# gam0022/hanamaru-renderer

Hardware: AMD Instinct MI355X
Metric: Mpaths/sec at 1920x1080x1024spp (rtcamp6 scene); achieved GB/s in BVH traversal (higher is better)
Workload: dtype f32

## Files before the change

hanamaru-renderer_amd/csrc/device_scene.h:

```cpp
#pragma once
#include <math.h>
#include <stdint.h>

#if defined(__HIPCC__)
#define HD __host__ __device__ __forceinline__
#else
#define HD inline
#endif

namespace hr {

struct alignas(16) f4 { float x, y, z, w; };

struct alignas(16) Node {
    float nearx, neary, farx, fary;
    float nearz, farz;
    uint32_t a;
    uint32_t b;
};
HD void node_set_box(Node &n, const float *mn, const float *mx, int octant) {
    n.nearx = (octant & 1) ? mx[0] : mn[0]; n.farx = (octant & 1) ? mn[0] : mx[0];
    n.neary = (octant & 2) ? mx[1] : mn[1]; n.fary = (octant & 2) ? mn[1] : mx[1];
    n.nearz = (octant & 4) ? mx[2] : mn[2]; n.farz = (octant & 4) ? mn[2] : mx[2];
}
// ... 174 lines not shown
    uint32_t tail_div;
    uint32_t wg_budget;
    GovDev *gov;
    uint64_t rec_lo_off;
    uint32_t org_x, org_y, reg_w, reg_h;
    const uint32_t *tile_list;
    uint32_t tile_count;
};
HD uint32_t rp_reg_w(const RenderParams &rp) { return rp.reg_w ? rp.reg_w : rp.width; }
HD uint32_t rp_reg_h(const RenderParams &rp) { return rp.reg_h ? rp.reg_h : rp.height; }
HD bool rp_in_region(const RenderParams &rp, uint32_t px, uint32_t py) { return px < rp_reg_w(rp) && py < rp_reg_h(rp); }

HD void tile_lane_pixel(const RenderParams &rp, uint32_t tile, uint32_t j, uint32_t &px, uint32_t &py, uint32_t &sub) {
    uint32_t tx = tile % rp.tiles_x, ty = tile / rp.tiles_x;
    uint32_t pix = j >> 2;
    sub = j & 3u;
    px = tx * 4u + (pix & 3u);
    py = ty * 4u + (pix >> 2);
}
HD void tile_lane_frame_pixel(const RenderParams &rp, uint32_t tile, uint32_t j, uint32_t &px, uint32_t &py, uint32_t &sub) {
    tile_lane_pixel(rp, tile, j, px, py, sub);
    px += rp.org_x;
    py += rp.org_y;
}

static const int ISAAC_TAIL = 64;
static const int REC_FLOATS = 32;
static const int REC_DRAWS = 28;
static const int REC_HEAD = 28;
static const int LENS_FAST = 5;
static const int DRAWS_PER_PATH = 20;
static const uint32_t REC_ITEM_FLOATS = 64u * REC_FLOATS;
static const int SEG_B1 = 11, SEG_B2 = 21, SEG_NBLK = 11;
HD uint32_t rec_slot(uint32_t lane_base, uint32_t slot) { return lane_base + (slot >> 2) * 256u + (slot & 3u); }

struct Counters {
    unsigned long long paths, rays, node_tests, tri_tests, sphere_tests, cuboid_tests, rng_overflow, shadow_culled;
    unsigned long long shade_calls, shade_lanes, box_passes, box_lanes, leaf_calls, leaf_lanes, outer_iters, pad2;
    unsigned long long phase_cycles[4];
    unsigned long long seed_phase[8];
};

}
```

hanamaru-renderer_amd/csrc/hr_api.hip:

```cpp
#include <hip/hip_runtime.h>

#include <cmath>
#include <cstdarg>
#include <cstdio>
#include <cstring>
#include <map>
#include <mutex>
#include <string>
#include <vector>

#include "bvh_build.h"
#include "device_scene.h"
#include "flatten.h"
#include "gpu_bvh.h"
#include "hanamaru_hip.h"
#include "hanamaru_hip_debug.h"
#include "hr_comm.h"
#include "isaac_core.h"
#include "post_core.h"
#include "pt_core.h"

using namespace hr;


// ... 87 lines not shown
    uint32_t ovf_cap = 0;
    u64 *ovf_win = nullptr;
    size_t draws_cap = 0;
    uint64_t rec_lo_off = 0;
    int draw_residuals = 1;
    u64 *ring = nullptr;
    int seed_split = 16;
    uint32_t init_prio = 1;
    hipEvent_t seed_done[2] = {nullptr, nullptr}, trace_done[2] = {nullptr, nullptr};
    bool seed_pending[2] = {false, false}, trace_pending[2] = {false, false};
    uint64_t batch_counter = 0;
    Counters *d_counters = nullptr;
    uint32_t *d_tile_counter = nullptr;
    bool counters = false;
    uint32_t batch = 0;
    uint32_t adv_den = 2, leaf_den = 2;
    int min_waves = 5;
    uint32_t trace_wgs = 6;
    uint32_t tail_div = 16;
    uint32_t trace_grid = 0, trace_budget = 0;
    uint32_t node_unroll = 2;
    uint32_t kchunk = 0;
    int trace_boost = -1;
    GovDev *gov = nullptr;
    bool quant_nodes = true;
    int max_leaf = 4;
    double split_ratio = -1.0;
    int bvh_builder = -1;
    int builder_in_use = 0;
    double bvh_build_ms = 0;
    uint64_t max_tail_bytes = 20ull << 30;
    int seed_mode = 2;
    int seed_prof = 0;
    uint32_t seed_prio = 3;
    uint32_t nee_cull = 7;
    uint32_t rr_start = 0;
    uint32_t ploc_top = hr::lbvh::PLOC_TOP_CLUSTERS;
    int trace_mode = 0;
    int trace_mode_opt = -1;
    int precise_opt = -1;
    bool precise = false;
    bool wf_has_prec = false;
    WfQueues wf{};
    void *wf_block = nullptr;
    uint32_t wf_adv_den = 2, wf_trav_wgs = 8, wf_shade_wgs = 8;
    int debug_skip = 0;
    std::vector<EventPair> seed_events, trace_events, post_events, debug_events;
    double seed_ms = 0, trace_ms = 0, post_ms = 0, debug_ms = 0;
    uint64_t seed_launches = 0, trace_launches = 0, debug_launches = 0;
    uint64_t paths_rendered = 0;
    std::vector<std::pair<uint64_t, hipEvent_t>> markers;
    uint64_t next_ticket = 1;
};

static std::mutex g_bound_mu;
static std::map<const void *, std::pair<const hr_ctx *, size_t>> g_bound;
static void unbind_accumulator(hr_ctx *c) {
    std::lock_guard<std::mutex> lk(g_bound_mu);
    for (auto it = g_bound.begin(); it != g_bound.end();) it = it->second.first == c ? g_bound.erase(it) : std::next(it);
}
static void free_scene(hr_ctx *c) {
    for (void *p : c->scene_allocs) (void)hipFree(p);
    c->scene_allocs.clear();
    c->have_scene = false;
}
template <class T>
// ... 746 lines not shown
    return HR_OK;
}
static int launch_split(hr_ctx *c, const RenderParams &rp, int slot, std::vector<hipEvent_t> *marks = nullptr, uint32_t *plog = nullptr, const WfQueues *queues = nullptr) {
    const WfQueues wq = queues ? *queues : c->wf;
    hipStream_t st = c->stream;
    auto mark = [&]() -> hipError_t { if (!marks) return hipSuccess; hipEvent_t e; hipError_t r = hipEventCreate(&e); if (r != hipSuccess) return r; marks->push_back(e); return hipEventRecord(e, st); };
    const bool log = plog != nullptr;
    const WfStartFn start = select_wf_start_kernel(c->precise, rp.tile_list != nullptr);
    const WfTraverseFn traverse = select_wf_traverse_kernel(c->counters, c->dsc.qnodes != nullptr, log);
    const WfShadeFn shade = select_wf_shade_kernel(c->counters, c->precise, log);
    if (!start || !traverse || !shade) return fail(HR_ERR_UNSUPPORTED, "split pipeline: no kernel instantiation for these options (kernel_variants.h)");
    HIP_TRY(hipMemsetAsync(wq.counts, 0, (WF_STEPS + 2) * WF_SUBQ * sizeof(WfCounts), st));
    HIP_TRY(mark());
    auto grid_of = [&](uint32_t wgs_per_cu) { return dim3(std::max<uint32_t>(16u, (uint32_t)c->num_cus * wgs_per_cu / 16u * 16u)); };
    hipLaunchKernelGGL(start, grid_of(8u), dim3(256), 0, st, c->dsc, rp, c->recs[slot], wq);
    HIP_TRY(mark());
    RenderParams rt = rp;
    rt.adv_den = c->wf_adv_den;
    const dim3 gt = grid_of(c->wf_trav_wgs), gs = grid_of(c->wf_shade_wgs), b(256);
    for (uint32_t step = 1; step <= WF_STEPS; step++) {
        hipLaunchKernelGGL(traverse, gt, b, 0, st, c->dsc, rt, wq, step, c->d_counters);
        HIP_TRY(mark());
        hipLaunchKernelGGL(shade, gs, b, 0, st, c->dsc, rp, c->recs[slot], wq, step, c->d_counters, plog);
        HIP_TRY(mark());
    }
    HIP_TRY(hipGetLastError());
    return HR_OK;
}

static int launch_seed(hr_ctx *c, const RenderParams &rp, int slot, hipStream_t st) {
    const bool list = rp.tile_list != nullptr;
    uint64_t paths = (uint64_t)(list ? rp.tile_count : rp.tiles_x * rp.tiles_y) * rp.num_k * 64u;
    uint32_t grid = (uint32_t)std::min<uint64_t>((paths + SEED_COLS - 1) / SEED_COLS, (uint64_t)c->num_cus);
    const SeedVariant *v = select_seed_kernel(c->seed_mode, c->seed_split, c->seed_prof, rp.rec_lo_off != 0, list);
    if (!v) return fail(HR_ERR_UNSUPPORTED, "no seed kernel instantiation for seed_mode %d, seed_split %d, seed_prof %d%s (kernel_variants.h)", c->seed_mode, c->seed_split, c->seed_prof, list ? " under a tile mask" : "");
    const bool skip = (c->debug_skip & 2) != 0;
    if (!skip && v->ring && !c->ring) HIP_TRY(hipMalloc((void **)&c->ring, (size_t)c->num_cus * SEED_RING_WORDS_MAX * sizeof(u64)));
    EventPair ev;
    HIP_TRY(timed_begin(ev, st));
    hipError_t e = hipSuccess;
    if (!skip) {
        RenderParams krp = rp;
        int lens_shape = c->dsc.cam.lens_shape;
        void *args[7] = {&krp, &lens_shape, &c->ring, &c->recs[slot], &c->ovf, &c->ovf_win, &c->d_counters};
        if (!v->ring) std::copy(args + 3, args + 7, args + 2);
        e = hipLaunchKernel(v->fn, dim3(grid), dim3(v->threads), args, SEED_LDS_BYTES, st);
    }
    HIP_TRY(timed_end(e, ev, st, c->seed_events, &c->seed_launches));
    return HR_OK;
}

static void target_params(const hr_ctx *c, RenderParams &rp) {
    rp.width = c->W; rp.height = c->H;
    rp.org_x = c->RX; rp.org_y = c->RY; rp.reg_w = c->RW; rp.reg_h = c->RH;
    rp.tiles_x = (c->RW + 3) / 4; rp.tiles_y = (c->RH + 3) / 4;
}
static void knob_params(const hr_ctx *c, RenderParams &rp) {
    rp.adv_den = c->adv_den; rp.leaf_den = c->leaf_den;
    rp.node_unroll = c->node_unroll; rp.kchunk = c->kchunk;
    rp.nee_cull_off = ~c->nee_cull & 7u;
}
static uint32_t render_batch(const hr_ctx *c, uint32_t tiles, bool split) {
    uint64_t batch = c->batch;
    if (!batch) {
        const uint64_t per_sampling_paths = (uint64_t)tiles * 64u;
        batch = std::min<uint64_t>(64, std::max<uint64_t>(4, (33177600ull + per_sampling_paths - 1) / per_sampling_paths));
    }
// ... 746 lines not shown
    constexpr OptionField(int hr_ctx::*p) : i(p) {}
};
enum { OPT_SYNC = 1, OPT_GOVERN = 2 };
struct OptionRow {
    const char *key;
    OptionField field;
    double lo, hi, step;
    const char *error;
    int flags;
};
static const OptionRow PRODUCT_OPTIONS[] = {
    {"counters", &hr_ctx::counters, 1, 0, 0, "", 0},
    {"batch", &hr_ctx::batch, 0, 64, 0, "batch must be in [1,64], or 0 for automatic", OPT_SYNC},
    {"trace_boost", &hr_ctx::trace_boost, -1, 4, 1, "trace_boost must be -1 (governed by the measured kernel times) or a level 0 .. 4", OPT_SYNC | OPT_GOVERN},
    {"precise_shading", &hr_ctx::precise_opt, -1, 1, 1, "precise_shading must be -1 (automatic), 0 or 1", OPT_SYNC | OPT_GOVERN},
    {"quant_nodes", &hr_ctx::quant_nodes, 1, 0, 0, "", 0},
    {"bvh_builder", &hr_ctx::bvh_builder, -1, 2, 1, "bvh_builder must be -1 (by scene size), 0 (host SAH), 1 (device LBVH) or 2 (device PLOC)", 0},
    {"max_leaf", &hr_ctx::max_leaf, 1, 15, 0, "max_leaf must be in [1,15]", 0},
};
static const OptionRow DEBUG_OPTIONS[] = {
    {"adv_den", &hr_ctx::adv_den, 1, 64, 0, "adv_den must be in [1,64]", 0},
    {"leaf_den", &hr_ctx::leaf_den, 1, 64, 0, "leaf_den must be in [1,64]", 0},
    {"min_waves", &hr_ctx::min_waves, 4, 6, 0, "min_waves must be in [4,6]", 0},
    {"kchunk", &hr_ctx::kchunk, 0, 64, 0, "kchunk must be in [1,64], or 0 for the default", 0},
    {"node_unroll", &hr_ctx::node_unroll, 1, 2, 1, "node_unroll must be 1 or 2", 0},
    {"tail_div", &hr_ctx::tail_div, 1, 0, 0, "", 0},
    {"trace_grid", &hr_ctx::trace_grid, 1, 0, 0, "", 0},
    {"trace_budget", &hr_ctx::trace_budget, 1, 0, 0, "", 0},
    {"trace_wgs", &hr_ctx::trace_wgs, 1, 8, 0, "trace_wgs must be in [1,8]", 0},
    {"seed_prio", &hr_ctx::seed_prio, 0, 3, 0, "seed_prio must be in [0,3]", 0},
    {"init_prio", &hr_ctx::init_prio, 0, 3, 0, "init_prio must be in [0,3]", 0},
    {"seed_split", &hr_ctx::seed_split, 8, 28, 4, "seed_split must be 8, 12, 16, 20, 24 or 28", 0},
    {"seed_prof", &hr_ctx::seed_prof, 1, 0, 0, "", 0},
    {"ploc_top", &hr_ctx::ploc_top, 1, 1 << 16, 0, "ploc_top must be in [1,65536]", 0},
    {"trace_mode", &hr_ctx::trace_mode_opt, -1, 1, 1, "trace_mode must be -1 (automatic), 0 (megakernel) or 1 (split: traversal kernel + shading kernel)", OPT_SYNC | OPT_GOVERN},
    {"draw_residuals", &hr_ctx::draw_residuals, 0, 1, 1, "draw_residuals must be 0 or 1", 0},
    {"wf_adv_den", &hr_ctx::wf_adv_den, 0, 64, 0, "wf_adv_den must be in [0,64]", 0},
    {"wf_trav_wgs", &hr_ctx::wf_trav_wgs, 1, 16, 0, "wf_trav_wgs must be in [1,16]", 0},
    {"wf_shade_wgs", &hr_ctx::wf_shade_wgs, 1, 16, 0, "wf_shade_wgs must be in [1,16]", 0},
    {"debug_skip", &hr_ctx::debug_skip, 1, 0, 0, "", 0},
};
static int apply_option(hr_ctx *c, const OptionRow &r, double value) {
    if (r.lo <= r.hi) {
        bool ok = !(value < r.lo || value > r.hi);
        if (ok && r.step > 0) ok = std::fmod(value - r.lo, r.step) == 0.0;
        if (!ok) return fail(HR_ERR_INVALID, "%s", r.error);
    }
    if (r.flags & OPT_SYNC) { int rc = sync_all(c); if (rc) return rc; }
    if (r.field.b) c->*r.field.b = value != 0.0;
    else if (r.field.u) c->*r.field.u = (uint32_t)value;
    else c->*r.field.i = (int)value;
    return r.flags & OPT_GOVERN ? govern_reset(c) : HR_OK;
}

static int set_plane_option(hr_ctx *c, double value, const Plane &p, const Plane &other, int (*off_first)(hr_ctx *)) {
    if (value != 0 && value != 1) return fail(HR_ERR_INVALID, "%s must be 0 or 1", p.option);
    if (value == 1 && !c->W) return fail(HR_ERR_NO_TARGET, "%s: hr_set_resolution not called", p.option);
    int rc = sync_all(c);
    if (rc) return rc;
    if (value == 0 || !(c->*p.on)) invalidate_denoised(c);
    if (value == 0) {
        c->*p.on = false;
        if ((rc = off_first(c))) return rc;
        return plane_free(c, p);
    }
    if (c->*p.on) return HR_OK;
// ... 242 lines not shown
```

hanamaru-renderer_amd/csrc/isaac_core.h:

```cpp
#pragma once
#include "device_scene.h"

namespace hr {

typedef unsigned long long u64;

#if defined(__HIPCC__)
#define HR_NOUNROLL _Pragma("unroll 1")
#define HR_UNROLL _Pragma("unroll")
#else
#define HR_NOUNROLL
#define HR_UNROLL
#endif

#define HR_ISAAC_MIX(a, b, c, d, e, f, g, h) \
    a -= e; f ^= h >> 9;  h += a;            \
    b -= f; g ^= a << 9;  a += b;            \
    c -= g; h ^= b >> 23; b += c;            \
    d -= h; a ^= c << 15; c += d;            \
    e -= a; b ^= d >> 14; d += e;            \
    f -= b; c ^= e << 20; e += f;            \
    g -= c; d ^= f >> 17; f += g;            \
    h -= d; e ^= g << 14; g += h;

// ... 74 lines not shown
    static_assert(0 < B1 && B1 < B2 && B2 < 32, "segment boundaries");
    u64 A = w.r[0] + s0, B = w.r[1] + s1, C = w.r[2] + s2, D = w.r[3] + s3, E = w.r[4], F = w.r[5], G = w.r[6], H = w.r[7];
    HR_NOUNROLL
    for (int i = 0; i < 32; i++) { HR_ISAAC_MIX_2(A, B, C, D, E, F, G, H) }
    u64 a = w.r[0] + s0, b = w.r[1] + s1, c = w.r[2] + s2, d = w.r[3] + s3, e = w.r[4], f = w.r[5], g = w.r[6], h = w.r[7];
    out.state(0, a, b, c, d, e, f, g, h, A, B, C, D, E, F, G, H);
    HR_NOUNROLL
    for (int i = 0; i < B1; i++) {
        HR_ISAAC_MIX_1(a, b, c, d, e, f, g, h)
        A += a; B += b; C += c; D += d; E += e; F += f; G += g; H += h;
        HR_ISAAC_MIX_2(A, B, C, D, E, F, G, H)
    }
    out.state(1, a, b, c, d, e, f, g, h, A, B, C, D, E, F, G, H);
    HR_NOUNROLL
    for (int i = B1; i < B2; i++) {
        HR_ISAAC_MIX_1(a, b, c, d, e, f, g, h)
        A += a; B += b; C += c; D += d; E += e; F += f; G += g; H += h;
        HR_ISAAC_MIX_2(A, B, C, D, E, F, G, H)
    }
    out.state(2, a, b, c, d, e, f, g, h, A, B, C, D, E, F, G, H);
}
template <int NBLK, class Mem>
HD void isaac_init_run(Mem &mem, const u64 *st16) {
    u64 a = st16[0], b = st16[1], c = st16[2], d = st16[3], e = st16[4], f = st16[5], g = st16[6], h = st16[7];
    u64 A = st16[8], B = st16[9], C = st16[10], D = st16[11], E = st16[12], F = st16[13], G = st16[14], H = st16[15];
    HR_NOUNROLL
    for (int i = 0; i < 8 * NBLK; i += 8) {
        HR_ISAAC_MIXB_1(a, b, c, d, e, f, g, h)
        A += a; B += b; C += c; D += d; E += e; F += f; G += g; H += h;
        HR_ISAAC_MIXB_2(A, B, C, D, E, F, G, H)
        mem.st(i, A); mem.st(i + 1, B); mem.st(i + 2, C); mem.st(i + 3, D);
        mem.st(i + 4, E); mem.st(i + 5, F); mem.st(i + 6, G); mem.st(i + 7, H);
    }
}

struct AheadRegs { u64 a, b, c, d, e, f, g, h, A, B, C, D, E, F, G, H; };
#define HR_AHEAD_BLOCK(r)                                                                           \
    HR_ISAAC_MIX_1(r.a, r.b, r.c, r.d, r.e, r.f, r.g, r.h)                                          \
    r.A += r.a; r.B += r.b; r.C += r.c; r.D += r.d; r.E += r.e; r.F += r.f; r.G += r.g; r.H += r.h; \
    HR_ISAAC_MIX_2(r.A, r.B, r.C, r.D, r.E, r.F, r.G, r.H)
template <int P1BLK, class Out>
HD void isaac_ahead_part1(Out &out, const IsaacWarm &w, u64 s0, u64 s1, u64 s2, u64 s3, AheadRegs &r) {
    r.A = w.r[0] + s0; r.B = w.r[1] + s1; r.C = w.r[2] + s2; r.D = w.r[3] + s3; r.E = w.r[4]; r.F = w.r[5]; r.G = w.r[6]; r.H = w.r[7];
    HR_NOUNROLL
    for (int i = 0; i < 32; i++) { HR_ISAAC_MIX_2(r.A, r.B, r.C, r.D, r.E, r.F, r.G, r.H) }
    r.a = w.r[0] + s0; r.b = w.r[1] + s1; r.c = w.r[2] + s2; r.d = w.r[3] + s3; r.e = w.r[4]; r.f = w.r[5]; r.g = w.r[6]; r.h = w.r[7];
    out.state(0, r.a, r.b, r.c, r.d, r.e, r.f, r.g, r.h, r.A, r.B, r.C, r.D, r.E, r.F, r.G, r.H);
    HR_NOUNROLL
    for (int i = 0; i < P1BLK; i++) { HR_AHEAD_BLOCK(r) }
}
template <int NRUN, int NBLK, int P1BLK, class Out>
HD void isaac_ahead_part2(Out &out, AheadRegs &r) {
    static_assert(NRUN * NBLK == 32 && P1BLK > 0 && P1BLK < NBLK, "runs tile the sweep; part 1 ends inside the first run");
    HR_NOUNROLL
    for (int i = P1BLK; i < NBLK; i++) { HR_AHEAD_BLOCK(r) }
    out.state(1, r.a, r.b, r.c, r.d, r.e, r.f, r.g, r.h, r.A, r.B, r.C, r.D, r.E, r.F, r.G, r.H);
    HR_NOUNROLL
    for (int k = 2; k < NRUN; k++) {
        HR_NOUNROLL
        for (int i = 0; i < NBLK; i++) { HR_AHEAD_BLOCK(r) }
        out.state(k, r.a, r.b, r.c, r.d, r.e, r.f, r.g, r.h, r.A, r.B, r.C, r.D, r.E, r.F, r.G, r.H);
    }
}

template <int TAILN, class Mem, class Tail>
HD void isaac_round(Mem &mem, Tail &tail);
// ... 269 lines not shown
```

hanamaru-renderer_amd/csrc/kernel_variants.h:

```cpp
#pragma once

#define HR_VARIANT(kernel, ...) {__VA_ARGS__, kernel<__VA_ARGS__>}
template <class Row, size_t N, class Match>
static const Row *find_row(const Row (&table)[N], Match match) {
    for (const Row &r : table)
        if (match(r)) return &r;
    return nullptr;
}
template <class Row>
static auto fn_of(const Row *r) -> decltype(r->fn) { return r ? r->fn : nullptr; }

typedef void (*TraceFn)(Scene, RenderParams, float *, Counters *, uint32_t *, uint32_t *);
struct TraceVariant { bool cnt; int minw; bool qn, rr, log, prec, list; TraceFn fn; };
static const TraceVariant TRACE_VARIANTS[] = {
    HR_VARIANT(trace_kernel, false, 5, true, false, false, false, false), HR_VARIANT(trace_kernel, false, 5, false, false, false, false, false),
    HR_VARIANT(trace_kernel, false, 4, true, false, false, false, false), HR_VARIANT(trace_kernel, false, 6, true, false, false, false, false),
    HR_VARIANT(trace_kernel, true, 3, true, false, false, false, false), HR_VARIANT(trace_kernel, true, 3, false, false, false, false, false),
    HR_VARIANT(trace_kernel, false, 5, true, true, false, false, false), HR_VARIANT(trace_kernel, false, 5, false, true, false, false, false),
    HR_VARIANT(trace_kernel, true, 3, true, true, false, false, false), HR_VARIANT(trace_kernel, true, 3, false, true, false, false, false),
    HR_VARIANT(trace_kernel, false, 4, true, false, false, true, false), HR_VARIANT(trace_kernel, false, 4, false, false, false, true, false),
    HR_VARIANT(trace_kernel, false, 5, true, false, false, true, false), HR_VARIANT(trace_kernel, false, 3, true, false, false, true, false),
    HR_VARIANT(trace_kernel, true, 3, true, false, false, true, false), HR_VARIANT(trace_kernel, true, 3, false, false, false, true, false),
    HR_VARIANT(trace_kernel, false, 3, true, false, true, false, false), HR_VARIANT(trace_kernel, false, 3, false, false, true, false, false),
    HR_VARIANT(trace_kernel, false, 3, true, false, true, true, false), HR_VARIANT(trace_kernel, false, 3, false, false, true, true, false),
// ... 35 lines not shown
}
static WfShadeFn select_wf_shade_kernel(bool counters, bool precise, bool log) {
    const bool cnt = counters && !log;
    return fn_of(find_row(WF_SHADE_VARIANTS, [&](const WfShadeVariant &r) { return r.cnt == cnt && r.prec == precise && r.log == log; }));
}

typedef void (*DebugRenderFn)(Scene, RenderParams, int, float *, Counters *);
struct DebugRenderVariant { bool cnt, qn; DebugRenderFn fn; };
static const DebugRenderVariant DEBUG_RENDER_VARIANTS[] = {HR_VARIANT(debug_render_kernel, false, true), HR_VARIANT(debug_render_kernel, false, false),
                                                           HR_VARIANT(debug_render_kernel, true, true), HR_VARIANT(debug_render_kernel, true, false)};
static DebugRenderFn select_debug_render_kernel(bool counters, bool qn) {
    return fn_of(find_row(DEBUG_RENDER_VARIANTS, [&](const DebugRenderVariant &r) { return r.cnt == counters && r.qn == qn; }));
}
typedef void (*GuideRenderFn)(Scene, RenderParams, float *);
struct GuideRenderVariant { bool qn; GuideRenderFn fn; };
static const GuideRenderVariant GUIDE_RENDER_VARIANTS[] = {HR_VARIANT(guide_render_kernel, true), HR_VARIANT(guide_render_kernel, false)};
static GuideRenderFn select_guide_render_kernel(bool qn) {
    return fn_of(find_row(GUIDE_RENDER_VARIANTS, [&](const GuideRenderVariant &r) { return r.qn == qn; }));
}
typedef void (*GuideChainFn)(Scene, RenderParams, uint32_t, float *);
struct GuideChainVariant { bool qn; GuideChainFn fn; };
static const GuideChainVariant GUIDE_CHAIN_VARIANTS[] = {HR_VARIANT(guide_chain_kernel, true), HR_VARIANT(guide_chain_kernel, false)};
static GuideChainFn select_guide_chain_kernel(bool qn) {
    return fn_of(find_row(GUIDE_CHAIN_VARIANTS, [&](const GuideChainVariant &r) { return r.qn == qn; }));
}
typedef void (*TraceDebugFn)(Scene, RenderParams, uint32_t, const float *, const float *, float *, int32_t *, Counters *);
struct TraceDebugVariant { bool qn, cnt; TraceDebugFn fn; };
static const TraceDebugVariant TRACE_DEBUG_VARIANTS[] = {HR_VARIANT(trace_debug_kernel, true, false), HR_VARIANT(trace_debug_kernel, false, false),
                                                         HR_VARIANT(trace_debug_kernel, true, true), HR_VARIANT(trace_debug_kernel, false, true)};
static TraceDebugFn select_trace_debug_kernel(bool counters, bool qn) {
    return fn_of(find_row(TRACE_DEBUG_VARIANTS, [&](const TraceDebugVariant &r) { return r.cnt == counters && r.qn == qn; }));
}

struct SeedVariant { int mode, split, prof; bool lo; const void *fn; uint32_t threads; bool ring; bool list = false; };
static const SeedVariant SEED_VARIANTS[] = {
    {0, 0, 0, false, (const void *)seed_isaac64_kernel, 64 * SEED_WAVES, false},
    {1, 8, 0, false, (const void *)seed_pc_kernel<8>, 256, true},
    {1, 12, 0, false, (const void *)seed_pc_kernel<12>, 256, true},
    {1, 16, 0, false, (const void *)seed_pc_kernel<16>, 256, true},
    {1, 20, 0, false, (const void *)seed_pc_kernel<20>, 256, true},
    {1, 24, 0, false, (const void *)seed_pc_kernel<24>, 256, true},
    {1, 28, 0, false, (const void *)seed_pc_kernel<28>, 256, true},
    {1, 16, 1, false, (const void *)seed_pc_kernel<16, true>, 256, true},
    {1, 20, 1, false, (const void *)seed_pc_kernel<20, true>, 256, true},
    {2, 0, 0, false, (const void *)seed_seg_kernel<false, false>, 256, true},
    {2, 0, 1, false, (const void *)seed_seg_kernel<true, false>, 256, true},
    {2, 0, 0, true, (const void *)seed_seg_kernel<false, true>, 256, true},
    {2, 0, 1, true, (const void *)seed_seg_kernel<true, true>, 256, true},
    {2, 0, 0, false, (const void *)seed_seg_kernel<false, false, true>, 256, true, true},
    {2, 0, 0, true, (const void *)seed_seg_kernel<false, true, true>, 256, true, true},
#if defined(HR_EXPERIMENTS)
    {3, 0, 0, false, (const void *)seed_ps_kernel<0>, 256, true},
    {3, 0, 1, false, (const void *)seed_ps_kernel<1>, 256, true},
    {3, 0, 2, false, (const void *)seed_ps_kernel<2>, 256, true},
    {3, 0, 3, false, (const void *)seed_ps_kernel<3>, 256, true},
    {4, 0, 0, false, (const void *)seed_w5_kernel<false>, 320, true},
    {4, 0, 1, false, (const void *)seed_w5_kernel<true>, 320, true},
#endif
};
static const SeedVariant *select_seed_kernel(int seed_mode, int seed_split, int seed_prof, bool twin, bool list = false) {
    int split = 0, prof = seed_prof ? 1 : 0;
    bool lo = false;
    if (seed_mode == 2) lo = twin;
    else if (seed_mode == 1) split = prof ? (seed_split == 20 ? 20 : 16) : seed_split;
    else if (seed_mode == 3) prof = seed_prof >= 1 && seed_prof <= 3 ? seed_prof : 0;
    else if (seed_mode == 0) prof = 0;
    return find_row(SEED_VARIANTS, [&](const SeedVariant &r) { return r.mode == seed_mode && r.split == split && r.prof == prof && r.lo == lo && r.list == list; });
}

typedef void (*AccumulateFn)(RenderParams, const float *, float *, double *, uint32_t *);
struct AccumulateVariant { bool mom, cnts, list; AccumulateFn fn; };
static const AccumulateVariant ACCUMULATE_VARIANTS[] = {HR_VARIANT(accumulate_kernel, false, false, false), HR_VARIANT(accumulate_kernel, true, false, false),
                                                        HR_VARIANT(accumulate_kernel, false, true, false),  HR_VARIANT(accumulate_kernel, true, true, false),
                                                        HR_VARIANT(accumulate_kernel, false, true, true),   HR_VARIANT(accumulate_kernel, true, true, true)};
static AccumulateFn select_accumulate_kernel(bool moments, bool counts, bool list) {
    return fn_of(find_row(ACCUMULATE_VARIANTS, [&](const AccumulateVariant &r) { return r.mom == moments && r.cnts == counts && r.list == list; }));
}
```

hanamaru-renderer_amd/csrc/seed_kernels.h:

```cpp
#pragma once
#include <hip/hip_runtime.h>

#include "adapt_core.h"
#include "device_scene.h"
#include "isaac_core.h"

using namespace hr;


__device__ __forceinline__ uint32_t lds_addr(const void *p) { return (uint32_t)(size_t)(const __attribute__((address_space(3))) void *)p; }
__device__ __forceinline__ u64 lds_load64(uint32_t a) { return *(const __attribute__((address_space(3))) u64 *)(size_t)a; }

static const int SEED_COLS = 80;
static const int SEED_WAVES = 2, SEED_LANES = SEED_COLS / SEED_WAVES;
__device__ __forceinline__ uint32_t seed_gov_begin(const RenderParams &rp, bool stamp) {
    if (!rp.gov) return rp.pad[1];
    const int32_t lvl = __hip_atomic_load(&rp.gov->level, __ATOMIC_RELAXED, __HIP_MEMORY_SCOPE_AGENT);
    if (stamp) {
        atomicMin(&rp.gov->t0[0][rp.gov_slot], (unsigned long long)__builtin_amdgcn_s_memrealtime());
        if (blockIdx.x == 0) rp.gov->lvl[0][rp.gov_slot] = (uint32_t)lvl;
    }
    return gov_producer_prio(lvl, rp.pad[1] & 3u);
}
__device__ __forceinline__ void seed_gov_end(const RenderParams &rp, bool stamp) {
// ... 338 lines not shown
        const u64x2 q[8] = {{a, b}, {c, d}, {e, f}, {g, h}, {A, B}, {C, D}, {E, F}, {G, H}};
#pragma unroll
        for (int j = 0; j < 8; j++) asm volatile("global_store_dwordx4 %0, %1, off sc1\n\ts_nop 1" : : "v"(dst + j * SEED_LANES), "v"(q[j]) : "memory");
    }
};
struct SegLane {
    uint32_t col, run;
    bool on;
};
__device__ __forceinline__ SegLane seg_lane(bool consumer, uint32_t lane) {
    SegLane l;
    if (lane < (uint32_t)SEED_LANES) { l.col = lane; l.run = consumer ? 2u : 0u; l.on = true; }
    else if (consumer) { l.col = lane - (uint32_t)SEED_LANES; l.run = 1u; l.on = true; }
    else { l.col = lane - 16u; l.run = 1u; l.on = lane < 56u; if (!l.on) l.col = (uint32_t)SEED_LANES - 1u; }
    return l;
}
struct SegRegs {
    typedef u64 u64x2_t __attribute__((ext_vector_type(2)));
    u64x2_t v[8];
    __device__ __forceinline__ void load(const u64 *ring_wg, uint64_t g, uint32_t half, const SegLane &l) {
        const u64 *regs = ring_wg + (g & (SEED_RING_GROUPS - 1)) * SegLayout::GROUP_WORDS + half * SegLayout::HALF_WORDS + (size_t)l.run * SegLayout::STATE_WORDS + (size_t)l.col * 2u;
#pragma unroll
        for (int q = 0; q < 8; q++) v[q] = __builtin_nontemporal_load(reinterpret_cast<const u64x2_t *>(regs + q * (2 * SEED_LANES)));
    }
    __device__ __forceinline__ void run(unsigned char *lds_half, const SegLane &l) const {
        u64 st16[16];
#pragma unroll
        for (int q = 0; q < 8; q++) { st16[2 * q] = v[q].x; st16[2 * q + 1] = v[q].y; }
        const uint32_t first = l.run == 0u ? 0u : l.run == 1u ? (uint32_t)SEG_B1 : (uint32_t)SEG_B2;
        LdsHalfMem m{reinterpret_cast<u64 *>(lds_half) + l.col + (size_t)first * 8u * SEED_LANES};
        if (l.on) isaac_init_run<SEG_NBLK>(m, st16);
    }
};
template <bool PROF, bool LO, bool LIST>
__device__ __forceinline__ void seed_seg_consumer(const RenderParams &rp, int lens_shape, const PcRange &r, unsigned char *smem, uint32_t lane, uint32_t half,
                                                  float *__restrict__ recs, uint32_t *__restrict__ ovf, u64 *__restrict__ win, Counters *cnt) {
    uint32_t *ovf_list = ovf + (size_t)(blockIdx.x * 2u + half) * rp.ovf_cap;
    uint32_t ovf_count = 0;
    unsigned long long pc[8] = {0, 0, 0, 0, 0, 0, 0, 0}, tm = 0;
#define HR_STAMP(i) do { if (PROF) { unsigned long long now_ = __builtin_readcyclecounter(); pc[i] += now_ - tm; tm = now_; } } while (0)
    const SegLane sl = seg_lane(true, lane);
    SegRegs regs;
    const uint32_t colr = lane < (uint32_t)SEED_LANES ? lane : 0u;
    unsigned char *lds_half = smem + (size_t)half * SEED_LDS_HALF_BYTES;
    LdsHalfMem m{reinterpret_cast<u64 *>(lds_half) + colr};
    const uint64_t n_groups = r.G1 - r.G0;
    __syncthreads();
    for (uint64_t it = 1; it <= n_groups; it++) {
        if (PROF) tm = __builtin_readcyclecounter();
        const uint64_t g = r.G0 + it - 1;
        if (it == 1) regs.load(r.ring_wg, g, half, sl);
        const uint64_t pid = g * SEED_COLS + half * SEED_LANES + colr;
        const bool in_range = pid < r.paths;
        const uint32_t item = (uint32_t)((in_range ? pid : r.paths - 1) >> 6), j = (uint32_t)((in_range ? pid : r.paths - 1) & 63u);
        uint32_t tile = item / rp.num_k;
        uint32_t px, py, sub;
        tile_lane_frame_pixel(rp, launch_tile<LIST>(rp, tile), j, px, py, sub);
        const bool valid = in_range && px < rp.width && py < rp.height;
        HR_STAMP(0);
        if (PROF) { __builtin_amdgcn_s_waitcnt(0x0F70); HR_STAMP(1); }
        regs.run(lds_half, sl);
        HR_STAMP(2);
        __syncthreads();
        HR_STAMP(3);
        if (it < n_groups) regs.load(r.ring_wg, r.G0 + it, half, sl);
        RecStore rs(recs, pid, rp.rec_lo_off);
        RecordTail<RecStore, LO> lt(rs, lens_shape);
        if (lane < (uint32_t)SEED_LANES) {
            isaac_round<REC_DRAWS>(m, lt);
            lt.finish();
        }
        HR_STAMP(4);
        ovf_note(lane < (uint32_t)SEED_LANES && valid && lt.overflow(), pid, ovf_list, ovf_count, rp.ovf_cap);
        HR_STAMP(5);
        if (PROF) pc[7]++;
        __syncthreads();
        HR_STAMP(6);
    }
#undef HR_STAMP
    if (PROF && lane == 0)
        for (int i = 0; i < 8; i++) atomicAdd(&cnt->seed_phase[i], pc[i]);
    const bool lane_on = lane < (uint32_t)SEED_LANES;
    seed_fixup_wave<LdsHalfMem, LO, LIST>(rp, lens_shape, m, colr, lane_on, ovf_list, ovf_count, win + (size_t)(blockIdx.x * 2u + half) * SEED_WIN_WORDS, recs, cnt);
}
template <bool LIST>
__device__ __forceinline__ void seed_seg_producer(const RenderParams &rp, const PcRange &r, unsigned char *smem, uint32_t lane, uint32_t half, const uint32_t pprio) {
    const IsaacWarm warm = isaac_warm();
    const SegLane sl = seg_lane(false, lane);
    SegRegs regs;
    unsigned char *lds_half = smem + (size_t)half * SEED_LDS_HALF_BYTES;
    const uint64_t n_groups = r.G1 - r.G0;
    uint64_t frontier = r.first_path & ~63ull;
    auto ahead = [&](uint64_t upto) {
        const uint64_t need = upto * SEED_COLS;
        for (; frontier < need && frontier < r.end_path; frontier += 64) {
            if (((frontier >> 6) & 1u) != half) continue;
            const uint64_t pid0 = frontier + lane;
            const bool on = pid0 >= r.first_path && pid0 < r.end_path && !(rp.pad[2] & 4u);
            const uint64_t ppid = pid0 >= r.first_path && pid0 < r.end_path ? pid0 : r.end_path - 1;
            const uint32_t item = (uint32_t)(ppid >> 6), j = (uint32_t)(ppid & 63u);
            uint32_t tile = item / rp.num_k, k = item - tile * rp.num_k;
            uint32_t px, py, sub;
            tile_lane_frame_pixel(rp, launch_tile<LIST>(rp, tile), j, px, py, sub);
            bool pvalid = px < rp.width && py < rp.height;
            u64 s, t;
            path_seed_words(rp.width, rp.height, pvalid ? px : 0u, pvalid ? py : 0u, sub, s, t);
            const uint64_t g = ppid / SEED_COLS;
            const uint32_t c80 = (uint32_t)(ppid - g * SEED_COLS), hh = c80 >= (uint32_t)SEED_LANES ? 1u : 0u;
            SegStateOut out{r.ring_wg + (g & (SEED_RING_GROUPS - 1)) * SegLayout::GROUP_WORDS + hh * SegLayout::HALF_WORDS + (size_t)(c80 - hh * (uint32_t)SEED_LANES) * 2u};
            if (on) isaac_init_ahead<SEG_B1, SEG_B2>(out, warm, 8700304ULL, (u64)(rp.sampling_begin + k * rp.stride), s, t);
        }
        __builtin_amdgcn_s_waitcnt(0);
    };
    ahead(r.G0 + 2);
    __syncthreads();
    if (n_groups >= 1) regs.load(r.ring_wg, r.G0, half, sl);
    for (uint64_t it = 1; it <= n_groups; it++) {
        regs.run(lds_half, sl);
        __syncthreads();
        if (it < n_groups) regs.load(r.ring_wg, r.G0 + it, half, sl);
        if (((pprio >> 2) & 3u) != (pprio & 3u)) {
            const uint32_t pr = (it & 1u) ? (pprio >> 2) & 3u : pprio & 3u;
            if (pr == 0u) __builtin_amdgcn_s_setprio(0); else if (pr == 1u) __builtin_amdgcn_s_setprio(1); else if (pr == 2u) __builtin_amdgcn_s_setprio(2); else __builtin_amdgcn_s_setprio(3);
        }
        ahead(r.G0 + it + 2);
        __syncthreads();
    }
}
template <bool PROF = false, bool LO = false, bool LIST = false>
__global__ __launch_bounds__(256) void seed_seg_kernel(RenderParams rp, int lens_shape, u64 *__restrict__ ring, float *__restrict__ recs,
                                                       uint32_t *__restrict__ ovf, u64 *__restrict__ win, Counters *cnt) {
    extern __shared__ __align__(16) unsigned char smem[];
    const uint32_t lane = threadIdx.x & 63u, wave = threadIdx.x >> 6, half = wave & 1u;
    const bool consumer = wave < 2u;
    const uint32_t pprio = consumer ? 0u : seed_gov_begin(rp, wave == 2u && lane == 0u);
    const uint32_t prio = consumer ? rp.pad[0] : pprio & 3u;
    switch (prio) {
        case 0: break;
        case 1: __builtin_amdgcn_s_setprio(1); break;
        case 2: __builtin_amdgcn_s_setprio(2); break;
        default: __builtin_amdgcn_s_setprio(3); break;
    }
    PcRange r;
    r.paths = (uint64_t)launch_tiles<LIST>(rp) * rp.num_k * 64u;
    const uint64_t groups = (r.paths + SEED_COLS - 1) / SEED_COLS;
    r.G0 = groups * blockIdx.x / gridDim.x; r.G1 = groups * (blockIdx.x + 1) / gridDim.x;
    r.first_path = r.G0 * SEED_COLS; r.end_path = r.G1 * SEED_COLS < r.paths ? r.G1 * SEED_COLS : r.paths;
    r.ring_wg = ring + (size_t)blockIdx.x * SEED_RING_WORDS_MAX;
    if (consumer) seed_seg_consumer<PROF, LO, LIST>(rp, lens_shape, r, smem, lane, half, recs, ovf, win, cnt);
    else {
        seed_seg_producer<LIST>(rp, r, smem, lane, half, pprio);
        seed_gov_end(rp, wave == 2u && lane == 0u);
    }
}

#if defined(HR_EXPERIMENTS)
static const int PS_NRUN = 4, PS_NBLK = 8, PS_P1BLK = 4;
struct PsLayout {
    static const size_t STATE_WORDS = (size_t)16 * SEED_LANES;
    static const size_t HALF_WORDS = PS_NRUN * STATE_WORDS;
    static const size_t GROUP_WORDS = 2 * HALF_WORDS;
};
static_assert(SEED_RING_GROUPS * PsLayout::GROUP_WORDS <= SEED_RING_WORDS_MAX, "the ring allocation of the producer / consumer kernel holds it");
struct PsStateOut {
    u64 *base;
    __device__ __forceinline__ void state(int k, u64 a, u64 b, u64 c, u64 d, u64 e, u64 f, u64 g, u64 h, u64 A, u64 B, u64 C, u64 D, u64 E, u64 F, u64 G, u64 H) {
        typedef u64 u64x2 __attribute__((ext_vector_type(2)));
        u64x2 *dst = reinterpret_cast<u64x2 *>(base + (size_t)k * PsLayout::STATE_WORDS);
        const u64x2 q[8] = {{a, b}, {c, d}, {e, f}, {g, h}, {A, B}, {C, D}, {E, F}, {G, H}};
#pragma unroll
        for (int j = 0; j < 8; j++) asm volatile("global_store_dwordx4 %0, %1, off sc1\n\ts_nop 1" : : "v"(dst + j * SEED_LANES), "v"(q[j]) : "memory");
    }
};
struct PsLane { uint32_t col, run; bool on; };
__device__ __forceinline__ PsLane ps_lane(uint32_t slot, uint32_t lane) {
    const uint32_t L = slot * 64u + lane;
    PsLane l;
    l.on = L < (uint32_t)(PS_NRUN * SEED_LANES);
    const uint32_t Lc = l.on ? L : 0u;
    l.run = Lc / (uint32_t)SEED_LANES; l.col = Lc - l.run * (uint32_t)SEED_LANES;
    return l;
}
struct PsRegs {
    typedef u64 u64x2_t __attribute__((ext_vector_type(2)));
// ... 378 lines not shown
```

Baseline: 1367.

## Add pre-run window to three-run ISAAC seed kernel producer

Adds a new seed-kernel form in which producer waves run the first few ISAAC blocks of the next group ahead of time, overlapping that work with the barrier wait. The producer keeps those results in registers and writes them to LDS after the barrier. The ring layout and run assignment change so producer and consumer lanes split the 32-block sweep into uneven runs. It also adds a producer-side cycle profiling variant. The new path is on by default through seed_prerun=1, at the cost of extra registers, one extra barrier at startup, and a more complex slot mapping.

```diff
diff --git a/hanamaru-renderer_amd/csrc/device_scene.h b/hanamaru-renderer_amd/csrc/device_scene.h
--- a/hanamaru-renderer_amd/csrc/device_scene.h
+++ b/hanamaru-renderer_amd/csrc/device_scene.h
@@ -230,6 +230,19 @@
 static const int DRAWS_PER_PATH = 20;
 static const uint32_t REC_ITEM_FLOATS = 64u * REC_FLOATS;
 static const int SEG_B1 = 11, SEG_B2 = 21, SEG_NBLK = 11;
+static const int SEGP_NBLK = 8, SEGP_PNBLK = 12, SEGP_PRE = 4, SEGP_XCOLS = 32, SEGP_AHEAD_END = 24;
+HD bool segp_wants(uint32_t col, int block) {
+    return block == 0 || block == 24 || (col < (uint32_t)SEGP_XCOLS ? block == 12 : block == 8 || block == 16);
+}
+HD uint32_t segp_slot(uint32_t col, int block) {
+    if (col < (uint32_t)SEGP_XCOLS) return block == 0 ? col : block == 12 ? 32u + col : 64u + col;
+    return 96u + (uint32_t)(block >> 3) * 8u + (col - (uint32_t)SEGP_XCOLS);
+}
+HD void segp_run(uint32_t slot, uint32_t &col, uint32_t &first, uint32_t &nblk) {
+    if (slot < 64u) { col = slot & 31u; first = (slot >> 5) * (uint32_t)SEGP_PNBLK; nblk = (uint32_t)SEGP_PNBLK; }
+    else if (slot < 96u) { col = slot - 64u; first = 24u; nblk = (uint32_t)SEGP_NBLK; }
+    else { col = (uint32_t)SEGP_XCOLS + ((slot - 96u) & 7u); first = ((slot - 96u) >> 3) * (uint32_t)SEGP_NBLK; nblk = (uint32_t)SEGP_NBLK; }
+}
 HD uint32_t rec_slot(uint32_t lane_base, uint32_t slot) { return lane_base + (slot >> 2) * 256u + (slot & 3u); }
 
 struct Counters {
diff --git a/hanamaru-renderer_amd/csrc/hr_api.hip b/hanamaru-renderer_amd/csrc/hr_api.hip
--- a/hanamaru-renderer_amd/csrc/hr_api.hip
+++ b/hanamaru-renderer_amd/csrc/hr_api.hip
@@ -143,6 +143,7 @@
     uint64_t max_tail_bytes = 20ull << 30;
     int seed_mode = 2;
     int seed_prof = 0;
+    int seed_prerun = 1;
     uint32_t seed_prio = 3;
     uint32_t nee_cull = 7;
     uint32_t rr_start = 0;
@@ -955,7 +956,7 @@
     const bool list = rp.tile_list != nullptr;
     uint64_t paths = (uint64_t)(list ? rp.tile_count : rp.tiles_x * rp.tiles_y) * rp.num_k * 64u;
     uint32_t grid = (uint32_t)std::min<uint64_t>((paths + SEED_COLS - 1) / SEED_COLS, (uint64_t)c->num_cus);
-    const SeedVariant *v = select_seed_kernel(c->seed_mode, c->seed_split, c->seed_prof, rp.rec_lo_off != 0, list);
+    const SeedVariant *v = select_seed_kernel(c->seed_mode, c->seed_split, c->seed_prof, rp.rec_lo_off != 0, list, c->seed_prerun != 0);
     if (!v) return fail(HR_ERR_UNSUPPORTED, "no seed kernel instantiation for seed_mode %d, seed_split %d, seed_prof %d%s (kernel_variants.h)", c->seed_mode, c->seed_split, c->seed_prof, list ? " under a tile mask" : "");
     const bool skip = (c->debug_skip & 2) != 0;
     if (!skip && v->ring && !c->ring) HIP_TRY(hipMalloc((void **)&c->ring, (size_t)c->num_cus * SEED_RING_WORDS_MAX * sizeof(u64)));
@@ -1768,6 +1769,7 @@
     {"init_prio", &hr_ctx::init_prio, 0, 3, 0, "init_prio must be in [0,3]", 0},
     {"seed_split", &hr_ctx::seed_split, 8, 28, 4, "seed_split must be 8, 12, 16, 20, 24 or 28", 0},
     {"seed_prof", &hr_ctx::seed_prof, 1, 0, 0, "", 0},
+    {"seed_prerun", &hr_ctx::seed_prerun, 0, 1, 1, "seed_prerun must be 1 (pre-run window of the three-run seed kernel) or 0 (its three equal runs)", OPT_SYNC},
     {"ploc_top", &hr_ctx::ploc_top, 1, 1 << 16, 0, "ploc_top must be in [1,65536]", 0},
     {"trace_mode", &hr_ctx::trace_mode_opt, -1, 1, 1, "trace_mode must be -1 (automatic), 0 (megakernel) or 1 (split: traversal kernel + shading kernel)", OPT_SYNC | OPT_GOVERN},
     {"draw_residuals", &hr_ctx::draw_residuals, 0, 1, 1, "draw_residuals must be 0 or 1", 0},
diff --git a/hanamaru-renderer_amd/csrc/isaac_core.h b/hanamaru-renderer_amd/csrc/isaac_core.h
--- a/hanamaru-renderer_amd/csrc/isaac_core.h
+++ b/hanamaru-renderer_amd/csrc/isaac_core.h
@@ -130,6 +130,42 @@
         mem.st(i, A); mem.st(i + 1, B); mem.st(i + 2, C); mem.st(i + 3, D);
         mem.st(i + 4, E); mem.st(i + 5, F); mem.st(i + 6, G); mem.st(i + 7, H);
     }
+}
+
+template <class Out>
+HD void isaac_init_ahead_pre(Out &out, const IsaacWarm &w, u64 s0, u64 s1, u64 s2, u64 s3) {
+    u64 A = w.r[0] + s0, B = w.r[1] + s1, C = w.r[2] + s2, D = w.r[3] + s3, E = w.r[4], F = w.r[5], G = w.r[6], H = w.r[7];
+    HR_NOUNROLL
+    for (int i = 0; i < 32; i++) { HR_ISAAC_MIX_2(A, B, C, D, E, F, G, H) }
+    u64 a = w.r[0] + s0, b = w.r[1] + s1, c = w.r[2] + s2, d = w.r[3] + s3, e = w.r[4], f = w.r[5], g = w.r[6], h = w.r[7];
+    out.state(0, a, b, c, d, e, f, g, h, A, B, C, D, E, F, G, H);
+#define HR_AHEAD_TO(from, to)                                                  \
+    HR_NOUNROLL                                                                \
+    for (int i = from; i < to; i++) {                                          \
+        HR_ISAAC_MIX_1(a, b, c, d, e, f, g, h)                                 \
+        A += a; B += b; C += c; D += d; E += e; F += f; G += g; H += h;        \
+        HR_ISAAC_MIX_2(A, B, C, D, E, F, G, H)                                 \
+    }                                                                          \
+    if (out.wants(to)) out.state(to, a, b, c, d, e, f, g, h, A, B, C, D, E, F, G, H);
+    HR_AHEAD_TO(0, 8)
+    HR_AHEAD_TO(8, 12)
+    HR_AHEAD_TO(12, 16)
+    HR_AHEAD_TO(16, 24)
+#undef HR_AHEAD_TO
+}
+template <int P>
+HD void isaac_init_prerun(u64 *st16, u64 (*kept)[8]) {
+    u64 a = st16[0], b = st16[1], c = st16[2], d = st16[3], e = st16[4], f = st16[5], g = st16[6], h = st16[7];
+    u64 A = st16[8], B = st16[9], C = st16[10], D = st16[11], E = st16[12], F = st16[13], G = st16[14], H = st16[15];
+    HR_UNROLL
+    for (int p = 0; p < P; p++) {
+        HR_ISAAC_MIX_1(a, b, c, d, e, f, g, h)
+        A += a; B += b; C += c; D += d; E += e; F += f; G += g; H += h;
+        HR_ISAAC_MIX_2(A, B, C, D, E, F, G, H)
+        kept[p][0] = A; kept[p][1] = B; kept[p][2] = C; kept[p][3] = D; kept[p][4] = E; kept[p][5] = F; kept[p][6] = G; kept[p][7] = H;
+    }
+    st16[0] = a; st16[1] = b; st16[2] = c; st16[3] = d; st16[4] = e; st16[5] = f; st16[6] = g; st16[7] = h;
+    st16[8] = A; st16[9] = B; st16[10] = C; st16[11] = D; st16[12] = E; st16[13] = F; st16[14] = G; st16[15] = H;
 }
 
 struct AheadRegs { u64 a, b, c, d, e, f, g, h, A, B, C, D, E, F, G, H; };
diff --git a/hanamaru-renderer_amd/csrc/kernel_variants.h b/hanamaru-renderer_amd/csrc/kernel_variants.h
--- a/hanamaru-renderer_amd/csrc/kernel_variants.h
+++ b/hanamaru-renderer_amd/csrc/kernel_variants.h
@@ -91,7 +91,7 @@
     return fn_of(find_row(TRACE_DEBUG_VARIANTS, [&](const TraceDebugVariant &r) { return r.cnt == counters && r.qn == qn; }));
 }
 
-struct SeedVariant { int mode, split, prof; bool lo; const void *fn; uint32_t threads; bool ring; bool list = false; };
+struct SeedVariant { int mode, split, prof; bool lo; const void *fn; uint32_t threads; bool ring; bool list = false; bool pre = false; };
 static const SeedVariant SEED_VARIANTS[] = {
     {0, 0, 0, false, (const void *)seed_isaac64_kernel, 64 * SEED_WAVES, false},
     {1, 8, 0, false, (const void *)seed_pc_kernel<8>, 256, true},
@@ -108,6 +108,14 @@
     {2, 0, 1, true, (const void *)seed_seg_kernel<true, true>, 256, true},
     {2, 0, 0, false, (const void *)seed_seg_kernel<false, false, true>, 256, true, true},
     {2, 0, 0, true, (const void *)seed_seg_kernel<false, true, true>, 256, true, true},
+    {2, 0, 2, false, (const void *)seed_seg_kernel<2, false>, 256, true},
+    {2, 0, 0, false, (const void *)seed_seg_kernel<false, false, false, true>, 256, true, false, true},
+    {2, 0, 1, false, (const void *)seed_seg_kernel<true, false, false, true>, 256, true, false, true},
+    {2, 0, 0, true, (const void *)seed_seg_kernel<false, true, false, true>, 256, true, false, true},
+    {2, 0, 1, true, (const void *)seed_seg_kernel<true, true, false, true>, 256, true, false, true},
+    {2, 0, 0, false, (const void *)seed_seg_kernel<false, false, true, true>, 256, true, true, true},
+    {2, 0, 0, true, (const void *)seed_seg_kernel<false, true, true, true>, 256, true, true, true},
+    {2, 0, 2, false, (const void *)seed_seg_kernel<2, false, false, true>, 256, true, false, true},
 #if defined(HR_EXPERIMENTS)
     {3, 0, 0, false, (const void *)seed_ps_kernel<0>, 256, true},
     {3, 0, 1, false, (const void *)seed_ps_kernel<1>, 256, true},
@@ -117,14 +125,14 @@
     {4, 0, 1, false, (const void *)seed_w5_kernel<true>, 320, true},
 #endif
 };
-static const SeedVariant *select_seed_kernel(int seed_mode, int seed_split, int seed_prof, bool twin, bool list = false) {
+static const SeedVariant *select_seed_kernel(int seed_mode, int seed_split, int seed_prof, bool twin, bool list = false, bool prerun = false) {
     int split = 0, prof = seed_prof ? 1 : 0;
-    bool lo = false;
-    if (seed_mode == 2) lo = twin;
+    bool lo = false, pre = false;
+    if (seed_mode == 2) { lo = twin; pre = prerun; if (seed_prof == 2) prof = 2; }
     else if (seed_mode == 1) split = prof ? (seed_split == 20 ? 20 : 16) : seed_split;
     else if (seed_mode == 3) prof = seed_prof >= 1 && seed_prof <= 3 ? seed_prof : 0;
     else if (seed_mode == 0) prof = 0;
-    return find_row(SEED_VARIANTS, [&](const SeedVariant &r) { return r.mode == seed_mode && r.split == split && r.prof == prof && r.lo == lo && r.list == list; });
+    return find_row(SEED_VARIANTS, [&](const SeedVariant &r) { return r.mode == seed_mode && r.split == split && r.prof == prof && r.lo == lo && r.list == list && r.pre == pre; });
 }
 
 typedef void (*AccumulateFn)(RenderParams, const float *, float *, double *, uint32_t *);
diff --git a/hanamaru-renderer_amd/csrc/seed_kernels.h b/hanamaru-renderer_amd/csrc/seed_kernels.h
--- a/hanamaru-renderer_amd/csrc/seed_kernels.h
+++ b/hanamaru-renderer_amd/csrc/seed_kernels.h
@@ -394,19 +394,89 @@
         if (l.on) isaac_init_run<SEG_NBLK>(m, st16);
     }
 };
-template <bool PROF, bool LO, bool LIST>
+struct SegpLayout {
+    static const size_t WAVE_WORDS = (size_t)16 * 64;
+    static const size_t HALF_WORDS = 2 * WAVE_WORDS;
+    static const size_t GROUP_WORDS = 2 * HALF_WORDS;
+};
+static_assert(SEED_RING_GROUPS * SegpLayout::GROUP_WORDS <= SEED_RING_WORDS_MAX, "the ring allocation of the producer / consumer kernel holds it");
+static_assert(2 * SEGP_XCOLS == 64 && SEGP_XCOLS + 4 * (SEED_LANES - SEGP_XCOLS) == 64, "64 producer runs and 64 consumer runs per half");
+static_assert(SEGP_PNBLK == SEGP_PRE + SEGP_NBLK && 2 * SEGP_PNBLK + SEGP_NBLK == 32 && 4 * SEGP_NBLK == 32 && SEGP_AHEAD_END == 32 - SEGP_NBLK, "the runs tile the sweep");
+struct SegpStateOut {
+    u64 *half;
+    uint32_t col;
+    __device__ __forceinline__ bool wants(int block) const { return segp_wants(col, block); }
+    __device__ __forceinline__ void state(int block, u64 a, u64 b, u64 c, u64 d, u64 e, u64 f, u64 g, u64 h, u64 A, u64 B, u64 C, u64 D, u64 E, u64 F, u64 G, u64 H) {
+        typedef u64 u64x2 __attribute__((ext_vector_type(2)));
+        const uint32_t s = segp_slot(col, block);
+        u64x2 *dst = reinterpret_cast<u64x2 *>(half + (size_t)(s >> 6) * SegpLayout::WAVE_WORDS + (size_t)(s & 63u) * 2u);
+        const u64x2 q[8] = {{a, b}, {c, d}, {e, f}, {g, h}, {A, B}, {C, D}, {E, F}, {G, H}};
+#pragma unroll
+        for (int j = 0; j < 8; j++) asm volatile("global_store_dwordx4 %0, %1, off sc1\n\ts_nop 1" : : "v"(dst + j * 64), "v"(q[j]) : "memory");
+    }
+};
+struct SegpLane {
+    uint32_t slot, col, first;
+};
+__device__ __forceinline__ SegpLane segp_lane(bool consumer, uint32_t lane) {
+    SegpLane l;
+    uint32_t nblk;
+    l.slot = (consumer ? 64u : 0u) + lane;
+    segp_run(l.slot, l.col, l.first, nblk);
+    return l;
+}
+struct SegpRegs {
+    typedef u64 u64x2_t __attribute__((ext_vector_type(2)));
+    u64x2_t v[8];
+    __device__ __forceinline__ void load(const u64 *ring_wg, uint64_t g, uint32_t half, const SegpLane &l) {
+        const u64 *regs = ring_wg + (g & (SEED_RING_GROUPS - 1)) * SegpLayout::GROUP_WORDS + half * SegpLayout::HALF_WORDS + (size_t)(l.slot >> 6) * SegpLayout::WAVE_WORDS + (size_t)(l.slot & 63u) * 2u;
+#pragma unroll
+        for (int q = 0; q < 8; q++) v[q] = __builtin_nontemporal_load(reinterpret_cast<const u64x2_t *>(regs + q * 128));
+    }
+    __device__ __forceinline__ void run(unsigned char *lds_half, const SegpLane &l) const {
+        u64 st16[16];
+#pragma unroll
+        for (int q = 0; q < 8; q++) { st16[2 * q] = v[q].x; st16[2 * q + 1] = v[q].y; }
+        LdsHalfMem m{reinterpret_cast<u64 *>(lds_half) + l.col + (size_t)l.first * 8u * SEED_LANES};
+        isaac_init_run<SEGP_NBLK>(m, st16);
+    }
+    __device__ __forceinline__ void prerun(u64 (*kept)[8]) {
+        u64 st16[16];
+#pragma unroll
+        for (int q = 0; q < 8; q++) { st16[2 * q] = v[q].x; st16[2 * q + 1] = v[q].y; }
+        isaac_init_prerun<SEGP_PRE>(st16, kept);
+#pragma unroll
+        for (int q = 0; q < 8; q++) { v[q].x = st16[2 * q]; v[q].y = st16[2 * q + 1]; }
+    }
+    __device__ __forceinline__ void finish(unsigned char *lds_half, const SegpLane &l, const u64 (*kept)[8]) const {
+        LdsHalfMem k{reinterpret_cast<u64 *>(lds_half) + l.col + (size_t)l.first * 8u * SEED_LANES};
+#pragma unroll
+        for (int p = 0; p < SEGP_PRE; p++)
+#pragma unroll
+            for (int j = 0; j < 8; j++) k.st(p * 8 + j, kept[p][j]);
+        u64 st16[16];
+#pragma unroll
+        for (int q = 0; q < 8; q++) { st16[2 * q] = v[q].x; st16[2 * q + 1] = v[q].y; }
+        LdsHalfMem m{k.col + (size_t)SEGP_PRE * 8u * SEED_LANES};
+        isaac_init_run<SEGP_NBLK>(m, st16);
+    }
+};
+template <bool PRE> struct SegForm { typedef SegLane Lane; typedef SegRegs Regs; static __device__ __forceinline__ Lane lane(bool consumer, uint32_t l) { return seg_lane(consumer, l); } };
+template <> struct SegForm<true> { typedef SegpLane Lane; typedef SegpRegs Regs; static __device__ __forceinline__ Lane lane(bool consumer, uint32_t l) { return segp_lane(consumer, l); } };
+template <bool PROF, bool LO, bool LIST, bool PRE>
 __device__ __forceinline__ void seed_seg_consumer(const RenderParams &rp, int lens_shape, const PcRange &r, unsigned char *smem, uint32_t lane, uint32_t half,
                                                   float *__restrict__ recs, uint32_t *__restrict__ ovf, u64 *__restrict__ win, Counters *cnt) {
     uint32_t *ovf_list = ovf + (size_t)(blockIdx.x * 2u + half) * rp.ovf_cap;
     uint32_t ovf_count = 0;
     unsigned long long pc[8] = {0, 0, 0, 0, 0, 0, 0, 0}, tm = 0;
 #define HR_STAMP(i) do { if (PROF) { unsigned long long now_ = __builtin_readcyclecounter(); pc[i] += now_ - tm; tm = now_; } } while (0)
-    const SegLane sl = seg_lane(true, lane);
-    SegRegs regs;
+    const typename SegForm<PRE>::Lane sl = SegForm<PRE>::lane(true, lane);
+    typename SegForm<PRE>::Regs regs;
     const uint32_t colr = lane < (uint32_t)SEED_LANES ? lane : 0u;
     unsigned char *lds_half = smem + (size_t)half * SEED_LDS_HALF_BYTES;
     LdsHalfMem m{reinterpret_cast<u64 *>(lds_half) + colr};
     const uint64_t n_groups = r.G1 - r.G0;
+    if (PRE) __syncthreads();
     __syncthreads();
     for (uint64_t it = 1; it <= n_groups; it++) {
         if (PROF) tm = __builtin_readcyclecounter();
@@ -445,11 +515,16 @@
     const bool lane_on = lane < (uint32_t)SEED_LANES;
     seed_fixup_wave<LdsHalfMem, LO, LIST>(rp, lens_shape, m, colr, lane_on, ovf_list, ovf_count, win + (size_t)(blockIdx.x * 2u + half) * SEED_WIN_WORDS, recs, cnt);
 }
-template <bool LIST>
-__device__ __forceinline__ void seed_seg_producer(const RenderParams &rp, const PcRange &r, unsigned char *smem, uint32_t lane, uint32_t half, const uint32_t pprio) {
+static const uint32_t SEG_PROF_FIT = 563u * SEGP_PRE;
+template <bool LIST, bool PRE, bool PROF>
+__device__ __forceinline__ void seed_seg_producer(const RenderParams &rp, const PcRange &r, unsigned char *smem, uint32_t lane, uint32_t half, const uint32_t pprio, Counters *cnt) {
     const IsaacWarm warm = isaac_warm();
-    const SegLane sl = seg_lane(false, lane);
-    SegRegs regs;
+    const typename SegForm<PRE>::Lane sl = SegForm<PRE>::lane(false, lane);
+    typename SegForm<PRE>::Regs regs;
+    u64 kept[PRE ? SEGP_PRE : 1][8];
+    uint32_t pc[8] = {0, 0, 0, 0, 0, 0, 0, 0}, tm = 0, chunks = 0;
+#define HR_NOW() __builtin_amdgcn_readfirstlane((uint32_t)__builtin_readcyclecounter())
+#define HR_STAMP(i) do { if (PROF) { const uint32_t now_ = HR_NOW(); pc[i] = __builtin_amdgcn_readfirstlane(pc[i] + (now_ - tm)); tm = now_; } } while (0)
     unsigned char *lds_half = smem + (size_t)half * SEED_LDS_HALF_BYTES;
     const uint64_t n_groups = r.G1 - r.G0;
     uint64_t frontier = r.first_path & ~63ull;
@@ -469,27 +544,60 @@
             path_seed_words(rp.width, rp.height, pvalid ? px : 0u, pvalid ? py : 0u, sub, s, t);
             const uint64_t g = ppid / SEED_COLS;
             const uint32_t c80 = (uint32_t)(ppid - g * SEED_COLS), hh = c80 >= (uint32_t)SEED_LANES ? 1u : 0u;
-            SegStateOut out{r.ring_wg + (g & (SEED_RING_GROUPS - 1)) * SegLayout::GROUP_WORDS + hh * SegLayout::HALF_WORDS + (size_t)(c80 - hh * (uint32_t)SEED_LANES) * 2u};
-            if (on) isaac_init_ahead<SEG_B1, SEG_B2>(out, warm, 8700304ULL, (u64)(rp.sampling_begin + k * rp.stride), s, t);
+            if constexpr (PRE) {
+                SegpStateOut out{r.ring_wg + (g & (SEED_RING_GROUPS - 1)) * SegpLayout::GROUP_WORDS + hh * SegpLayout::HALF_WORDS, c80 - hh * (uint32_t)SEED_LANES};
+                if (on) isaac_init_ahead_pre(out, warm, 8700304ULL, (u64)(rp.sampling_begin + k * rp.stride), s, t);
+            } else {
+                SegStateOut out{r.ring_wg + (g & (SEED_RING_GROUPS - 1)) * SegLayout::GROUP_WORDS + hh * SegLayout::HALF_WORDS + (size_t)(c80 - hh * (uint32_t)SEED_LANES) * 2u};
+                if (on) isaac_init_ahead<SEG_B1, SEG_B2>(out, warm, 8700304ULL, (u64)(rp.sampling_begin + k * rp.stride), s, t);
+            }
+            if (PROF) chunks = __builtin_amdgcn_readfirstlane(chunks + 1u);
         }
         __builtin_amdgcn_s_waitcnt(0);
     };
     ahead(r.G0 + 2);
-    __syncthreads();
-    if (n_groups >= 1) regs.load(r.ring_wg, r.G0, half, sl);
+    if constexpr (PRE) {
+        __syncthreads();
+        regs.load(r.ring_wg, r.G0, half, sl);
+        regs.prerun(kept);
+        __syncthreads();
+    } else {
+        __syncthreads();
+        if (n_groups >= 1) regs.load(r.ring_wg, r.G0, half, sl);
+    }
     for (uint64_t it = 1; it <= n_groups; it++) {
-        regs.run(lds_half, sl);
-        __syncthreads();
+        if (PROF) { tm = HR_NOW(); chunks = 0; }
+        if constexpr (PRE) regs.finish(lds_half, sl, kept);
+        else regs.run(lds_half, sl);
+        HR_STAMP(0);
+        __syncthreads();
+        HR_STAMP(1);
         if (it < n_groups) regs.load(r.ring_wg, r.G0 + it, half, sl);
         if (((pprio >> 2) & 3u) != (pprio & 3u)) {
             const uint32_t pr = (it & 1u) ? (pprio >> 2) & 3u : pprio & 3u;
             if (pr == 0u) __builtin_amdgcn_s_setprio(0); else if (pr == 1u) __builtin_amdgcn_s_setprio(1); else if (pr == 2u) __builtin_amdgcn_s_setprio(2); else __builtin_amdgcn_s_setprio(3);
         }
         ahead(r.G0 + it + 2);
-        __syncthreads();
-    }
-}
-template <bool PROF = false, bool LO = false, bool LIST = false>
+        if constexpr (PRE) regs.prerun(kept);
+        HR_STAMP(2);
+        __syncthreads();
+        if (PROF) {
+            const uint32_t now_ = HR_NOW(), wait = now_ - tm;
+            tm = now_;
+            const bool busy = chunks != 0;
+            pc[3] = __builtin_amdgcn_readfirstlane(pc[3] + (busy ? wait : 0u));
+            pc[4] = __builtin_amdgcn_readfirstlane(pc[4] + (busy ? 0u : wait));
+            pc[5] = __builtin_amdgcn_readfirstlane(pc[5] + (busy ? 1u : 0u));
+            pc[6] = __builtin_amdgcn_readfirstlane(pc[6] + (busy && wait < SEG_PROF_FIT ? 1u : 0u));
+            pc[7] = __builtin_amdgcn_readfirstlane(pc[7] + 1u);
+        }
+    }
+#undef HR_STAMP
+#undef HR_NOW
+    if (PROF && lane == 0)
+        for (int i = 0; i < 8; i++) atomicAdd(&cnt->seed_phase[i], (unsigned long long)pc[i]);
+}
+template <int PROF = 0, bool LO = false, bool LIST = false, bool PRE = false>
 __global__ __launch_bounds__(256) void seed_seg_kernel(RenderParams rp, int lens_shape, u64 *__restrict__ ring, float *__restrict__ recs,
                                                        uint32_t *__restrict__ ovf, u64 *__restrict__ win, Counters *cnt) {
     extern __shared__ __align__(16) unsigned char smem[];
@@ -509,9 +617,9 @@
     r.G0 = groups * blockIdx.x / gridDim.x; r.G1 = groups * (blockIdx.x + 1) / gridDim.x;
     r.first_path = r.G0 * SEED_COLS; r.end_path = r.G1 * SEED_COLS < r.paths ? r.G1 * SEED_COLS : r.paths;
     r.ring_wg = ring + (size_t)blockIdx.x * SEED_RING_WORDS_MAX;
-    if (consumer) seed_seg_consumer<PROF, LO, LIST>(rp, lens_shape, r, smem, lane, half, recs, ovf, win, cnt);
+    if (consumer) seed_seg_consumer<PROF == 1, LO, LIST, PRE>(rp, lens_shape, r, smem, lane, half, recs, ovf, win, cnt);
     else {
-        seed_seg_producer<LIST>(rp, r, smem, lane, half, pprio);
+        seed_seg_producer<LIST, PRE, PROF == 2>(rp, r, smem, lane, half, pprio, cnt);
         seed_gov_end(rp, wave == 2u && lane == 0u);
     }
 }
```

New measurement: 1417, median of 6. 3.6% higher.
